# dyouakim/smpl

Hardware: AMD Instinct MI355X
Metric: successor evaluations/sec, ManipLattice GetSuccs loop body (7-DOF arm, 256^3 voxel grid) (higher is better)
Workload: dtype f64; 1 GPU; cfg2: 7-DOF arm7, 256^3 grid @ 0.02 m, tabletop + 64 boxes (seed 2), frontier batch B=4096 open states x M=25 primitives, eps 5 ARA* frontier; fork semantics (xy rotation by state[3]); batch_states=4096, primitives=25, grid=256, queries=1, parallelism=single query

## Files before the change

### smpl_amd/capi.py

```python
from __future__ import annotations

import ctypes as C
import os

import numpy as np

from . import build as _build

_dp = C.POINTER(C.c_double)
_ip = C.POINTER(C.c_int32)
_up = C.POINTER(C.c_uint8)
_u64p = C.POINTER(C.c_uint64)

SYMBOLS = [
    "smplx_last_error", "smplx_device_count", "smplx_shard_range", "smplx_grid_create", "smplx_grid_destroy", "smplx_model_create",
    "smplx_model_destroy", "smplx_model_counts", "smplx_model_joints", "smplx_model_nodes", "smplx_model_pairs",
    "smplx_space_create", "smplx_space_destroy", "smplx_space_num_vars", "smplx_space_num_prims",
    "smplx_space_discretization", "smplx_cc_state_valid_batch", "smplx_cc_edge_valid_batch", "smplx_cc_interpolate",
    "smplx_cc_sphere_positions", "smplx_set_goal_joint", "smplx_set_goal_xyz", "smplx_goal_pose",
    "smplx_heuristic_batch", "smplx_bfs_size", "smplx_bfs_copy", "smplx_bfs_levels", "smplx_expand_batch",
    "smplx_expand_work_bytes", "smplx_expand_batch_device", "smplx_set_start", "smplx_start_id", "smplx_goal_id",
    "smplx_get_succs", "smplx_hint_frontier", "smplx_get_goal_heuristic", "smplx_num_states", "smplx_get_state",
    "smplx_plan", "smplx_expansion_log_size", "smplx_expansion_log", "smplx_extract_path", "smplx_post_process_path", "smplx_space_specialized", "smplx_model_const_header", "smplx_profile_begin",
    "smplx_profile_end", "smplx_counters_bytes", "smplx_counters_read", "smplx_plan_multi",
# ... 566 lines not shown
        lib().smplx_test_set_one_launch.argtypes = [C.c_void_p, C.c_int]
        _chk(lib().smplx_test_set_one_launch(self.h, int(mode)))

    def one_launch_steps(self):
        lib().smplx_test_one_launch_steps.argtypes = [C.c_void_p]
        lib().smplx_test_one_launch_steps.restype = C.c_longlong
        return int(lib().smplx_test_one_launch_steps(self.h))

    def step_counters_zero(self, stream=None):
        lib().smplx_test_step_counters_zero.argtypes = [C.c_void_p, C.c_void_p]
        r = lib().smplx_test_step_counters_zero(self.h, C.c_void_p(stream))
        if r < 0:
            _chk(r)
        return r == 1

    def set_search_capacity(self, states):
        lib().smplx_test_set_search_capacity.argtypes = [C.c_void_p, C.c_int]
        _chk(lib().smplx_test_set_search_capacity(self.h, int(states)))

    def plan(self, eps0, eps_final, eps_delta, improve=True, bounded=False, max_init=0, max_rep=0, cap=100000):
        P = SearchParams(eps0, eps_final, eps_delta, int(improve), int(bounded), max_init, max_rep)
        S = SearchStats()
        ids = np.zeros(cap, np.int32)
        _chk(lib().smplx_plan(self.h, C.byref(P), _p(ids, _ip), cap, C.byref(S)))
        n = lib().smplx_expansion_log_size(self.h)
        log = np.zeros(n, np.int32)
        if n:
            _chk(lib().smplx_expansion_log(self.h, _p(log, _ip)))
        out = {f: getattr(S, f) for f, _ in SearchStats._fields_}
        out["path"] = ids[:S.path_len].copy()
# ... 83 lines not shown
```

### smpl_amd/csrc/device_table.h

```cpp
#pragma once

#include <cstring>
#include <vector>

#include "kernels.h"
#include "space.h"

namespace {

int table_alloc(smplx_space* s, size_t cap)
{
    if (s->dt.d_table) (void)hipFree(s->dt.d_table);
    s->dt.d_table = nullptr;
    const int stride = smplx_table_stride(s->N);
    HIP_TRY(hipMalloc((void**)&s->dt.d_table, cap * (size_t)stride * sizeof(int32_t)));
    HIP_TRY(hipMemsetAsync(s->dt.d_table, 0, cap * (size_t)stride * sizeof(int32_t), s->stream));
    s->dt.cap = cap;
    s->hs.table.slots = s->dt.d_table;
    s->hs.table.mask = (uint32_t)(cap - 1);
    s->hs.table.stride = stride;
    s->hs.table.pad = 0;
    return SMPLX_OK;
}

// ... 36 lines not shown
{
    if (items.empty()) return SMPLX_OK;
    const int n = (int)(items.size() / ((size_t)lead->N + 2));
    if (int e = dbuf.reserve(items.size())) return e;
    if (int e = pbuf.reserve(items.size())) return e;
    std::memcpy(pbuf.p, items.data(), items.size() * sizeof(int32_t));
    HIP_TRY(hipMemcpyAsync(dbuf.p, pbuf.p, items.size() * sizeof(int32_t), hipMemcpyHostToDevice, stream));
    hipLaunchKernelGGL(k_table_insert, dim3(blocks_for(n, SMPLX_BLOCK)), dim3(SMPLX_BLOCK), 0, stream, lead->d_space, stab, dbuf.p, n, lead->N);
    HIP_TRY(hipGetLastError());
    return SMPLX_OK;
}

int table_ensure(smplx_space* s)
{
    if (s->dt.d_table) return SMPLX_OK;
    size_t cap = (size_t)1 << 18;
    const size_t nstates = s->lat.h_of_id.size();
    while (nstates * 2 > cap) cap *= 4;
    if (int e = table_realloc(s, cap)) return e;
    s->dt.count = nstates > 0 ? nstates - 1 : 0;
    return SMPLX_OK;
}

int table_flush(smplx_space* s, hipStream_t stream)
{
    if (!s->dt.d_table) return SMPLX_OK;
    if (int e = table_grow_if_needed(s)) return e;
    if (s->dt.pending_ins.empty()) return SMPLX_OK;
    std::vector<int32_t> items;
    table_take_pending(s, 0, items);
    return table_upload(s, items, s->dt.b_ins, s->dt.p_ins, stream, nullptr);
// ... 4 lines not shown
```

### smpl_amd/csrc/engine.hip

```cpp
#include <hip/hip_runtime.h>

#include <algorithm>
#include <chrono>
#include <cmath>
#include <cstdlib>
#include <cstring>
#include <functional>
#include <limits>
#include <memory>
#include <string>
#include <vector>

#include "../../include/smpl_amd.h"
#include "det_math.h"
#include "device_types.h"
#include "kernels.h"
#include "model_compile.h"
#include "specialize.h"
#include "test_hooks.h"
#include "host_core.h"
#include "grid_handle.h"
#include "lattice.h"
#include "space.h"
#include "bfs_host.h"
// ... 350 lines not shown
long long smplx_test_one_launch_steps(const smplx_space* s) { return s ? (long long)s->step.one_launch_steps : -1; }

int smplx_test_step_counters_zero(smplx_space* s, void* stream)
{
    if (!s) return set_error(SMPLX_E_ARG, "null space");
    for (StepLaunch::WorkCounters& w : s->step.work_counters) {
        if (w.stream != (hipStream_t)stream) continue;
        std::vector<int32_t> h(SMPLX_WORK_COUNTER_BYTES / sizeof(int32_t));
        HIP_TRY(hipStreamSynchronize(w.stream));
        HIP_TRY(hipMemcpy(h.data(), w.p, SMPLX_WORK_COUNTER_BYTES, hipMemcpyDeviceToHost));
        for (int32_t v : h) if (v != 0) return 0;
        return 1;
    }
    return set_error(SMPLX_E_ARG, "no step has run on this stream");
}

int smplx_test_set_search_helper(smplx_space* s, int on)
{
    if (!s) return set_error(SMPLX_E_ARG, "null space");
    s->ds.test_no_helper = on == 0;
    return SMPLX_OK;
}

int smplx_test_set_search_capacity(smplx_space* s, int states)
{
    if (!s || states < 0) return set_error(SMPLX_E_ARG, "bad argument");
    s->ds.test_capacity = states;
    return SMPLX_OK;
}

// ... 1116 lines not shown
```

### smpl_amd/csrc/kernels.h

```cpp
#pragma once

#ifndef __HIPCC_RTC__
#include <hip/hip_runtime.h>
#include <stdint.h>
#endif

#include "device_types.h"

#define SMPLX_BLOCK 128
#define SMPLX_SETUP_BLOCK (SMPLX_BLOCK + 64)
#define SMPLX_STEP_BLOCK SMPLX_SETUP_BLOCK
#define SMPLX_STEP_STATES 16
#define SMPLX_STEP_CTR_BASE 512
#define SMPLX_STEP_CTR_OVERFLOW (SMPLX_STEP_CTR_BASE + 64 * SMPLX_CMP_SHARDS)
#define SMPLX_STEP_CTR_DONE (SMPLX_STEP_CTR_OVERFLOW + 32)
#define SMPLX_WORK_COUNTER_BYTES 16384
#define SMPLX_SEARCH_STATIC_LDS (44 * 1024)
#define SMPLX_GLOBAL_AS __attribute__((address_space(1)))
#define SMPLX_TALLIES 6

static inline int smplx_small_block(int nprims) { return ((nprims * 7 + 1) + 63) / 64 * 64 + 64; }
static inline int smplx_search_block(int nprims) { const int b = smplx_small_block(nprims); return b + 64 <= 512 ? b + 64 : b; }
static inline size_t smplx_lds_bytes_n(size_t blob_bytes, int nroot, int nslots, int nvars, int stack_bytes, int nthreads)
{
    return blob_bytes + (size_t)(3 * nroot + 12 * nslots + nvars) * 8 * nthreads + (size_t)stack_bytes * nthreads;
}
static inline size_t smplx_lds_bytes(size_t blob_bytes, int nroot, int nslots, int nvars, int stack_bytes)
{
    return smplx_lds_bytes_n(blob_bytes, nroot, nslots, nvars, stack_bytes, SMPLX_BLOCK);
}

static inline int smplx_step_states(int nprims) { return (SMPLX_BLOCK - 2 + nprims) / nprims + 1; }

#define SMPLX_PER_ROBOT_KERNELS(X) \
    X(STATE_PREP, k_state_prep) X(EXPAND, k_expand) X(PIPE_PREP, k_pipe_prep) X(PIPE_SETUP, k_pipe_setup) \
    X(PIPE_CONFIGS, k_pipe_configs) X(PIPE_FINISH, k_pipe_finish) X(SMALL_BATCH, k_small_batch) X(EDGE_VALID, k_edge_valid) \
    X(STATE_VALID, k_state_valid) X(HEURISTIC, k_heuristic) X(SPHERE_POSITIONS, k_sphere_positions) X(SEARCH, k_search) \
    X(ATTACHED_POSITIONS, k_attached_positions) X(PLANNING_POSE, k_planning_pose) X(STEP_BLOCK, k_step_block)

extern "C" {
__global__ void k_state_prep(const SmplxSpaceDev* S, const double* Q, int B, double* goal_dist,
                             unsigned char* parent_valid, int* parent_lookups,
                         const SmplxSpaceDev* const* stab, const unsigned short* state_q);
__global__ void k_expand(const SmplxSpaceDev* S, const double* Q, int B, const double* goal_dist,
                         const unsigned char* parent_valid, const int* parent_lookups, unsigned char* out_flags,
                         int* out_coord, double* out_q, int* out_h, int* out_cost, int* out_lookups,
                         unsigned long long* counters, const int* deferred_count,
// ... 59 lines not shown
```

### smpl_amd/csrc/lattice_steps.h

```cpp
#pragma once

#include "bfs_record.h"
#include "model_lds.h"
#include "sphere_checks.h"

__device__ __forceinline__ void planning_fk(const ModelLds* __restrict__ M, const double* __restrict__ q, double p[3], double* R)
{
    double T[12];
#pragma unroll
    for (int i = 0; i < 12; ++i) T[i] = 0.0;
#ifdef SMPLX_CONST_MODEL
    const_planning_chain<0, true>(M, q, T);
#else
    bool first = true;
    const int nj = M->njoints;
    for (int j = 0; j < nj; ++j) {
        JointPtr jt = &M->joints[j];
        if (!jt->on_chain) continue;
        double qv = 0.0;
        if (jt->var >= 0) {
            qv = q[jt->var];
            if (MV_TYPE(M, jt->var) == SMPLX_JT_CONTINUOUS) qv = smplx_normalize_angle(qv);
        }
        apply_joint(jt, qv, T, first);
// ... 108 lines not shown
}

__device__ __forceinline__ int var_to_coord(const ModelLds* __restrict__ M, int v, double x)
{
    const double delta = MV_COORD_DELTA(M, v);
    const int ty = MV_TYPE(M, v);
    if (ty == SMPLX_JT_CONTINUOUS) {
        const double pos = smplx_normalize_angle_positive(x);
        int c = (int)((pos + delta * 0.5) / delta);
        if (c == MV_COORD_VALS(M, v)) c = 0;
        return c;
    }
    return (int)(((x - MV_MIN(M, v)) / delta) + 0.5);
}

template <bool ConcurrentInserts>
__device__ __forceinline__ int table_lookup(const SmplxTableDev& T, const int* __restrict__ c, int nv)
{
    if (!T.slots) return -1;
    unsigned int i = smplx_coord_hash(c, nv) & T.mask;
    while (true) {
        const SMPLX_GLOBAL_AS int* sl = as_global(T.slots) + (size_t)i * T.stride;
        const int tag = ConcurrentInserts ? __atomic_load_n(&sl[0], __ATOMIC_ACQUIRE) : __atomic_load_n(&sl[0], __ATOMIC_RELAXED);
        if (tag <= 0) return -1;
        bool same = true;
        for (int v = 0; v < nv; ++v) same = same && (ConcurrentInserts ? __atomic_load_n(&sl[1 + v], __ATOMIC_RELAXED) : sl[1 + v]) == c[v];
        if (same) return tag - 1;
        i = (i + 1) & T.mask;
    }
}

__device__ __forceinline__ void table_insert_item(const SmplxSpaceDev* __restrict__ S, const SmplxSpaceDev* const* __restrict__ stab,
                                                  const int* __restrict__ it, int nvars)
{
    const SmplxTableDev T = (stab ? stab[it[0]] : S)->table;
    if (!T.slots) return;
    const int id = it[1];
    int c[SMPLX_MAX_VARS];
    for (int v = 0; v < nvars; ++v) c[v] = it[2 + v];
    unsigned int k = smplx_coord_hash(c, nvars) & T.mask;
    while (true) {
// ... 19 lines not shown
{
    if ((int)blockIdx.x < first_block) return false;
    const int i = ((int)blockIdx.x - first_block) * (int)blockDim.x + (int)threadIdx.x;
    const int nvars = S->model.nvars;
    if (i < n) table_insert_item(S, stab, items + (size_t)i * (nvars + 2), nvars);
    return true;
}

extern "C" __global__ void __launch_bounds__(BLOCK)
k_table_insert(const SmplxSpaceDev* __restrict__ S, const SmplxSpaceDev* const* __restrict__ stab, const int* __restrict__ items,
               int n, int nvars)
{
    table_insert_items(S, stab, items, n, nvars);
}

__device__ __forceinline__ bool mprim_active(const SmplxActionsDev& A, double goal_dist, int type)
{
    if (type == SMPLX_MP_LONG) {
        if (A.use_long_and_short) return true;
        const bool near_goal = goal_dist <= A.thresh[SMPLX_MP_SHORT];
        return !(A.enabled[SMPLX_MP_SHORT] && near_goal);
    } else if (type == SMPLX_MP_SHORT) {
        if (A.use_long_and_short) return A.enabled[type] != 0;
        const bool near_goal = goal_dist <= A.thresh[type];
        return A.enabled[type] && near_goal;
    }
    return A.enabled[type] && goal_dist <= A.thresh[type];
}

__device__ __forceinline__ bool prim_has_action(const SmplxActionsDev& A, const SmplxGoalDev& G, int p)
{
    const int ty = A.type[p];
    return ty == SMPLX_MP_LONG || ty == SMPLX_MP_SHORT || (ty == SMPLX_MP_SNAP_XYZ_RPY && G.type == SMPLX_GOAL_JOINT);
}

__device__ __forceinline__ bool successor_values(const ModelLds* __restrict__ M, const SmplxActionsDev& A, const SmplxGoalDev& G,
                                                 int pi, const double* __restrict__ parent, double* __restrict__ sq)
{
    const int nv = MV_NVARS(M);
    const int type = A.type[pi];
    if (type == SMPLX_MP_LONG || type == SMPLX_MP_SHORT) {
        double d0 = A.delta[pi][0], d1 = nv > 1 ? A.delta[pi][1] : 0.0;
// ... 54 lines not shown
```

### smpl_amd/csrc/search_kernel.h

```cpp
#pragma once

#include "small_batch.h"

#define SMPLX_AC_LEVELS 16
#define SMPLX_AC_SLOTS 128
#define SMPLX_INFINITECOST 1000000000u

enum { SA_EVAL = 0, SA_SKIP = 1, SA_REORDER = 2, SA_EXIT = 3 };

struct SearchLds {
    int action;
    int buf;
    int seq;
    int helper_gave_up;
    int go;
    double reorder_eps;
    int reorder_size, reorder_dups;
    int ac_nlev;
    int ac_lo[SMPLX_AC_LEVELS + 1], ac_hi[SMPLX_AC_LEVELS + 1], ac_base[SMPLX_AC_LEVELS + 1];
    unsigned long long ac_val[SMPLX_AC_SLOTS];
};

typedef unsigned long long hent_t;
#define HENT_ABSENT (~0ull)
// ... 182 lines not shown
    return h;
}

__device__ __forceinline__ void sstate_reinit(SmplxSState& s, int call_number)
{
    s.g = SMPLX_INFINITECOST;
    s.f = SMPLX_INFINITECOST;
    s.eg = SMPLX_INFINITECOST;
    s.iteration_closed = 0;
    s.call_number = (unsigned short)call_number;
    s.bp = -1;
    s.heap_index = 0;
    s.flags = 0;
}

typedef int __attribute__((ext_vector_type(4))) sk_int4;

__device__ __forceinline__ void sstate_store(SMPLX_GLOBAL_AS SmplxSState* dst, const SmplxSState& s, bool with_heap_index)
{
    sk_int4 a;
    a.x = (int)s.g; a.y = (int)s.h; a.z = (int)s.f; a.w = (int)s.eg;
    *(SMPLX_GLOBAL_AS sk_int4*)dst = a;
    dst->bp = s.bp;
    if (with_heap_index) dst->heap_index = s.heap_index;
    *(SMPLX_GLOBAL_AS unsigned int*)&dst->iteration_closed = (unsigned int)s.iteration_closed | ((unsigned int)s.call_number << 16);
    dst->flags = s.flags;
}
__device__ __forceinline__ SmplxSState sstate_load(const SMPLX_GLOBAL_AS SmplxSState* src)
{
    const sk_int4 a = ((const SMPLX_GLOBAL_AS sk_int4*)src)[0], b = ((const SMPLX_GLOBAL_AS sk_int4*)src)[1];
    SmplxSState s;
    s.g = (unsigned int)a.x; s.h = (unsigned int)a.y; s.f = (unsigned int)a.z; s.eg = (unsigned int)a.w;
    s.bp = b.x; s.heap_index = b.y;
    s.iteration_closed = (unsigned short)((unsigned int)b.z & 0xFFFFu); s.call_number = (unsigned short)((unsigned int)b.z >> 16);
    s.flags = (unsigned int)b.w;
    return s;
}

struct TableProbe { int id; unsigned int free_slot; };
#define SMPLX_TABLE_WORDS ((SMPLX_MAX_VARS + 1 + 3) / 4)
static_assert(4 * SMPLX_TABLE_WORDS >= SMPLX_MAX_VARS + 1, "the words of a probe hold the tag and every coordinate of the widest robot");
static_assert(4 * SMPLX_TABLE_WORDS <= (SMPLX_MAX_VARS + 1 + 7) / 8 * 8, "... and lie inside its slot (smplx_table_stride)");
struct TableProbeLoads { sk_int4 w[SMPLX_TABLE_WORDS]; unsigned int slot; };
__device__ __forceinline__ void table_slot_load(const SmplxTableDev& T, unsigned int slot, int nv, sk_int4 w[SMPLX_TABLE_WORDS])
{
    const SMPLX_GLOBAL_AS sk_int4* sl = (const SMPLX_GLOBAL_AS sk_int4*)(as_global(T.slots) + (size_t)slot * T.stride);
    const int nw = (nv + 1 + 3) / 4;
#pragma unroll
    for (int k = 0; k < SMPLX_TABLE_WORDS; ++k) if (k < nw) w[k] = sl[k];
}
__device__ __forceinline__ bool table_slot_match(const sk_int4 w[SMPLX_TABLE_WORDS], const LDS_AS int* c, int nv)
{
    const int nw = (nv + 1 + 3) / 4;
    bool same = w[0].x > 0;
#pragma unroll
    for (int k = 0; k < SMPLX_TABLE_WORDS; ++k) {
        if (k >= nw) continue;
        const int base = 4 * k - 1;
        if (k > 0 && base < nv) same = same && w[k].x == c[base];
        if (base + 1 < nv) same = same && w[k].y == c[base + 1];
        if (base + 2 < nv) same = same && w[k].z == c[base + 2];
        if (base + 3 < nv) same = same && w[k].w == c[base + 3];
    }
    return same;
}
__device__ __forceinline__ TableProbeLoads table_probe_start(const SmplxTableDev& T, int nv, unsigned int hash)
{
    TableProbeLoads r;
    r.slot = hash & T.mask;
    table_slot_load(T, r.slot, nv, r.w);
    return r;
}
__device__ __forceinline__ TableProbe table_probe_finish(const SmplxTableDev& T, TableProbeLoads& ld, const LDS_AS int* c, int nv)
{
    TableProbe r;
    while (true) {
        if (ld.w[0].x == 0) { r.id = -1; r.free_slot = ld.slot; return r; }
        if (table_slot_match(ld.w, c, nv)) { r.id = ld.w[0].x - 1; r.free_slot = 0; return r; }
        ld.slot = (ld.slot + 1) & T.mask;
        table_slot_load(T, ld.slot, nv, ld.w);
    }
}
__device__ __forceinline__ void table_store_own(const SmplxTableDev& T, unsigned int slot, const LDS_AS int* c, int nv, int id)
{
    SMPLX_GLOBAL_AS int* sl = as_global(T.slots) + (size_t)slot * T.stride;
    for (int v = 0; v < nv; ++v) sl[1 + v] = c[v];
    sl[0] = id + 1;
}

__device__ __forceinline__ bool ancestor_cache_fill(const HeapRef& H, SearchLds& W, int lane, int n, int cnt)
{
    int nlev = 0, total = 0;
    int my_idx[2] = {-1, -1};
// ... 871 lines not shown
```

### smpl_amd/csrc/space.h

```cpp
#pragma once

#include <chrono>
#include <cstdint>
#include <memory>
#include <string>
#include <utility>
#include <vector>

#include "device_types.h"
#include "grid_handle.h"
#include "host_core.h"
#include "lattice.h"
#include "model_compile.h"
#include "specialize.h"

namespace {

struct OutView {
    double* sq = nullptr;
    int32_t* coord = nullptr;
    int32_t* h = nullptr;
    int32_t* id = nullptr;
    unsigned char* flags = nullptr;
    size_t bytes = 0;
// ... 18 lines not shown
    DevBuf<unsigned char> b_work, b_out;
    DevBuf<int32_t> b_cost, b_lookups;
    PinBuf<double> p_q;
    PinBuf<unsigned short> p_stateq;
    PinBuf<unsigned char> p_out;
    std::vector<int32_t> ins_items;
    OutView dv, pv;
    hipEvent_t done = nullptr;
    bool zero_copy = false;
    std::chrono::steady_clock::time_point t_issue;
};

struct DeviceTable {
    int32_t* d_table = nullptr;
    size_t cap = 0, count = 0;
    int64_t regrows = 0;
    std::vector<int32_t> pending_ins;
    DevBuf<int32_t> b_ins;
    PinBuf<int32_t> p_ins;
};

struct BfsHost {
    int32_t* d_dist = nullptr;
    int32_t* d_queue = nullptr;
    int32_t* d_counts = nullptr;
    int32_t* d_brick_queued = nullptr;
    int bricks[3] = {0, 0, 0};
    int64_t total = 0;
    int64_t ints = 0;
    bool reset_due = false;
// ... 166 lines not shown
```

### smpl_amd/csrc/step.h

```cpp
#pragma once

#include <algorithm>
#include <chrono>
#include <cstddef>
#include <cstdlib>
#include <cstring>
#include <functional>
#include <string>
#include <utility>
#include <vector>

#include "device_table.h"
#include "kernels.h"
#include "space.h"

namespace {

inline size_t counter_words(int B, int M) { return (size_t)blocks_for((long long)B * M, SMPLX_BLOCK) * SMPLX_TALLIES; }

struct ExpandWork {
    double* goal_dist;
    int32_t* state_lookups;
    unsigned char* state_bad;
    int32_t* edge_w;
// ... 81 lines not shown
inline size_t small_lds_bytes(const smplx_space* s)
{
    return smplx_lds_bytes_n(s->blob_bytes, s->lds_nroot, s->model.dev.nslots, s->model.dev.nvars, s->model.dev.stack_bytes,
                             smplx_small_block(s->M));
}

ExpandPath expand_path(const smplx_space* s, int B, int zero_copy_max, bool force_pipeline)
{
    const bool small = !s->step.fused_mode && B <= s->small.batch_max && smplx_small_block(s->M) <= 512 &&
                       small_lds_bytes(s) <= 150 * 1024 && s->step.work_list_items == 0 && s->small.pipeline_left == 0 &&
                       s->step.prof_used + 3 > s->step.prof_events.size();
    if (small && B <= zero_copy_max && s->step.prof_events.empty()) return ExpandPath::SmallZeroCopy;
    if (small && !force_pipeline) return ExpandPath::Small;
    if (s->step.fused_mode) return ExpandPath::Fused;
    const bool can_run = s->step.one_launch_blocks > 0 && !s->step.pipe_prep && s->step.work_list_items == 0 &&
                         s->step.prof_used + 3 > s->step.prof_events.size();
    const bool by_rule = s->ks.specialized && s->step.one_launch_per_cu >= 4 &&
                         blocks_for((long long)B * s->M, SMPLX_BLOCK) <= s->step.one_launch_blocks;
    if (can_run && s->step.one_launch != 0 && (s->step.one_launch == 1 || by_rule)) return ExpandPath::OneLaunch;
    return ExpandPath::Pipeline;
}

int step_block_resident(const smplx_space* s, size_t lds, int* blocks_per_cu)
{
    *blocks_per_cu = 0;
    if (smplx_step_states(s->M) > SMPLX_STEP_STATES) return 0;
    int per_cu = 0, cus = 0;
    const smplx::KernelRef& k = s->ks.k[smplx::K_STEP_BLOCK];
    const hipError_t e = k.fn ? hipModuleOccupancyMaxActiveBlocksPerMultiprocessor(&per_cu, k.fn, SMPLX_STEP_BLOCK, lds)
                              : hipOccupancyMaxActiveBlocksPerMultiprocessor(&per_cu, k.generic, SMPLX_STEP_BLOCK, lds);
    if (e != hipSuccess) { (void)hipGetLastError(); return 0; }
// ... 15 lines not shown
    *out = &s->step.work_counters.back();
    return SMPLX_OK;
}

int launch_expand(smplx_space* s, const ExpandArgs& a)
{
    const int B = a.B;
    ExpandWork k = carve_work(a.work, B, s->M, s->N);
    int32_t* d_id = a.k5 ? a.k5->d_id : nullptr;
    SmplxCompactDev cmp;
    std::memset(&cmp, 0, sizeof(cmp));
    if (a.k5 && a.k5->cmp) cmp = *a.k5->cmp;
    const ExpandPath path = expand_path(s, B, a.zero_copy ? B : 0, a.force_pipeline || cmp.rec_a);
    if (s->step.one_launch == 1 && path == ExpandPath::Pipeline)
        return set_error(SMPLX_E_ARG, "the one-launch step was asked for (smplx_test_set_one_launch) but cannot run: a pipeline test hook or a "
                                      "profile-event triple is set, or a block of k_step_block does not fit this model");
    const int32_t* ins_items = a.k5 && s->dt.d_table ? a.k5->items : nullptr;
    const int n_ins = ins_items ? a.k5->n_items : 0;
    if (s->step.work_list_items > 0) k.capacity = s->step.work_list_items;
    hipEvent_t* ev = nullptr;
    if (s->step.prof_used + 3 <= s->step.prof_events.size()) { ev = &s->step.prof_events[s->step.prof_used]; s->step.prof_used += 3; }
    const int bs = blocks_for(B, SMPLX_BLOCK);
    const int be = blocks_for((long long)B * s->M, SMPLX_BLOCK);
    if (path == ExpandPath::SmallZeroCopy || path == ExpandPath::Small) {
        ++s->small.small_launches;
        const ZeroCopy* zc = path == ExpandPath::SmallZeroCopy ? a.zero_copy : nullptr;
        const int small_block = smplx_small_block(s->M);
        KLAUNCH(s, K_SMALL_BATCH, k_small_batch, dim3(B + blocks_for(n_ins, small_block)), dim3(small_block), small_lds_bytes(s), a.stream, s->d_space,
                           zc ? zc->q : a.q, B, k.goal_dist,
                           k.state_bad, k.state_lookups, a.flags, a.coord, a.sq, a.h, a.cost, a.lookups, a.stab, a.state_q,
                           zc ? zc->flags : (unsigned char*)nullptr, zc ? zc->coord : (int32_t*)nullptr,
// ... 361 lines not shown
```

### smpl_amd/csrc/step_block.h

```cpp
#pragma once

#include "step_kernels.h"

extern "C" __global__ void __launch_bounds__(SMPLX_STEP_BLOCK)
k_step_block(const SmplxSpaceDev* __restrict__ S, const double* __restrict__ Q, int B,
             unsigned char* __restrict__ out_flags, int* out_coord, double* out_q,
             int* __restrict__ out_h, int* __restrict__ out_cost, int* __restrict__ out_lookups,
             unsigned long long* __restrict__ counters,
        const SmplxSpaceDev* const* __restrict__ stab, const unsigned short* __restrict__ state_q,
             int* __restrict__ out_id, SmplxCompactDev cmp, int* __restrict__ step_ctr, int nprims, int nvars,
             const unsigned char* __restrict__ blob, int blob_bytes)
{
    extern __shared__ __align__(16) unsigned char smem[];
    constexpr int NT = SMPLX_STEP_BLOCK;
#ifdef SMPLX_CONST_MODEL
    constexpr bool RS = true;
#else
    constexpr bool RS = false;
#endif
    __shared__ double s_gd[SMPLX_STEP_STATES];
    __shared__ int s_slk[SMPLX_STEP_STATES], s_sbad[SMPLX_STEP_STATES];
    __shared__ int s_W[BLOCK], s_pre[BLOCK], s_elk[BLOCK], s_ebad[BLOCK];
    __shared__ int s_wsum[BLOCK / 64];
#ifdef SMPLX_CONST_MODEL
// ... 6 lines not shown
    const SmplxActionsDev& A = S->actions;
    const int nv = ARG_NVARS(nvars);
    const long long n_edges = (long long)B * nprims;
    const long long e0 = (long long)blockIdx.x * BLOCK;
    const long long e1 = e0 + BLOCK - 1 < n_edges ? e0 + BLOCK - 1 : n_edges - 1;
    const int s0 = (int)(e0 / nprims), s1 = (int)(e1 / nprims);
    const int n_states = s1 - s0 + 1;
    const bool dist_wave = t >= BLOCK;
    const int l = t - BLOCK;
    const long long tid = e0 + t;
    const bool in_range = !dist_wave && tid < n_edges;
    const int si = in_range ? (int)(tid / nprims) : s0;
    const int pi = in_range ? (int)(tid - (long long)si * nprims) : 0;
    const int ks = si - s0;
    const SmplxSpaceDev* Sq = stab ? stab[state_q[si]] : S;
    const int type = A.type[pi];
    if (t < BLOCK) { s_elk[t] = 0; s_ebad[t] = 0; }
    if (t < SMPLX_STEP_STATES) { s_slk[t] = 0; s_sbad[t] = 0; }
#ifdef SMPLX_CONST_MODEL
    double pqv[CM_NV], sqv[CM_NV];
#pragma unroll
    for (int v = 0; v < CM_NV; ++v) { pqv[v] = 0.0; sqv[v] = 0.0; }
    if (in_range) {
#pragma unroll
        for (int v = 0; v < CM_NV; ++v) pqv[v] = Q[(int64_t)si * CM_NV + v];
    }
    for (int i = t; i < n_states * CM_NV; i += NT) s_pq[i] = Q[(int64_t)s0 * CM_NV + i];
#endif
    ModelLds Mv;
    ThreadLds L = setup_lds(S, smem, &Mv, NT, !RS, blob, blob_bytes, fetched);
    const ModelLds* M = &Mv;
    const SmplxGridDev grid = S->grid;
    int W = 0;
    int flags = SMPLX_F_INACTIVE;
    int succ_h = 0, succ_id = -1;
    bool succ_goal = false;
#ifdef SMPLX_CONST_MODEL
    int scv[CM_NV];
#pragma unroll
    for (int v = 0; v < CM_NV; ++v) scv[v] = 0;
    if (in_range) flags = pipe_edge_values(M, A, Sq, pi, pqv, sqv, W);
    if (dist_wave) {
        if constexpr (CM_PARENT_TRIG) {
            constexpr int PER = 64 / CM_NV;
            const int ls = l / CM_NV, lv = l - ls * CM_NV;
            for (int r0 = 0; r0 < n_states; r0 += PER) {
                const int k = r0 + ls;
                double ns = 0.0, nc = 0.0;
                if (ls < PER && k < n_states) {
                    const double x = s_pq[k * CM_NV + lv];
                    double rs = 0.0, rc = 0.0;
                    if ((CM_TRIG_ANY >> lv) & 1u) smplx_sincos(x, &rs, &rc);
                    ns = rs; nc = rc;
                    bool cont = false;
#pragma unroll
                    for (int u = 0; u < CM_NV; ++u) if (CM_VAR_TYPE[u] == SMPLX_JT_CONTINUOUS) cont = cont || lv == u;
// ... 25 lines not shown
            double qd[CM_NV];
#pragma unroll
            for (int v = 0; v < CM_NV; ++v) qd[v] = s_pq[l * CM_NV + v];
            s_gd[l] = metric_goal_distance(M, grid, bfs, qd);
        }
    }
#else
    if (dist_wave && l < n_states) {
        const SmplxBfsDev bfs = (stab ? stab[state_q[s0 + l]] : S)->bfs;
        s_gd[l] = metric_goal_distance(M, grid, bfs, Q + (int64_t)(s0 + l) * nv);
    }
#endif
    __syncthreads();
    int items = 0;
    if (in_range) {
        if (!mprim_active(A, s_gd[ks], type)) {
            flags = SMPLX_F_INACTIVE;
            W = 0;
        } else {
#ifdef SMPLX_CONST_MODEL
            if (flags != SMPLX_F_INACTIVE) {
#pragma unroll
                for (int v = 0; v < CM_NV; ++v) { s_sq[v * BLOCK + t] = sqv[v]; out_q[tid * CM_NV + v] = sqv[v]; }
            }
#ifndef ABL_NO_SUCC
            if (flags == 0) {
                constexpr bool SC = CM_PARENT_TRIG && CM_TRIG_PLANNING != 0;
                if constexpr (SC) {
                    double prow[2 * CM_NV], sn[CM_NV], cs[CM_NV];
#pragma unroll
                    for (int j = 0; j < 2 * CM_NV; ++j) prow[j] = s_trig[ks * SMPLX_TRIG_ROW + 2 * CM_NV + j];
                    parent_trig<CM_TRIG_PLANNING, true>(sqv, pqv, prow, sn, cs);
                    pipe_successor<true>(M, Sq, grid, sqv, scv, out_id != nullptr, succ_h, succ_id, succ_goal, sn, cs);
                } else {
                    pipe_successor(M, Sq, grid, sqv, scv, out_id != nullptr, succ_h, succ_id, succ_goal);
                }
            }
#endif
#else
            flags = pipe_edge_values(M, A, Sq, pi, Q + (int64_t)si * nv, out_q + tid * nv, W);
#endif
        }
        items = W > 0 ? W - 1 : 0;
    }
    const int lane = t & 63, wv = t >> 6;
    int incl = items;
    for (int off = 1; off < 64; off <<= 1) {
        const int u = __shfl_up(incl, off);
        if (lane >= off) incl += u;
    }
    if (!dist_wave) {
// ... 95 lines not shown
#endif
                h = succ_h;
                cost = A.cost[pi];
                flags = SMPLX_F_VALID | (succ_goal ? SMPLX_F_GOAL : 0);
            }
        } else {
            succ_id = -1;
        }
        out_flags[tid] = (unsigned char)flags;
        out_h[tid] = h;
        out_cost[tid] = cost;
        out_lookups[tid] = lookups;
        succ_h = h;
        if (out_id) out_id[tid] = succ_id;
    }
    if (cmp.rec_a) {
        __shared__ int c_cnt[BLOCK / 64][2];
        __shared__ int c_base[2];
        const bool is_a = in_range && (flags & SMPLX_F_VALID) != 0;
        const bool is_b = is_a && (succ_id < 0 || (flags & SMPLX_F_GOAL) != 0);
        const unsigned long long m_a = __ballot(is_a), m_b = __ballot(is_b);
        const unsigned long long below = lane == 0 ? 0ull : (~0ull >> (64 - lane));
        if (lane == 0 && !dist_wave) { c_cnt[wv][0] = __popcll(m_a); c_cnt[wv][1] = __popcll(m_b); }
        __syncthreads();
        if (t == 0) {
            int ta = 0, tb = 0;
#pragma unroll
            for (int k = 0; k < BLOCK / 64; ++k) { ta += c_cnt[k][0]; tb += c_cnt[k][1]; }
            const int shard = blockIdx.x % SMPLX_CMP_SHARDS;
            const int sa = cmp.cap_a / SMPLX_CMP_SHARDS, sb = cmp.cap_b / SMPLX_CMP_SHARDS;
            int ba = ta > 0 ? atomicAdd(&step_ctr[SMPLX_STEP_CTR_BASE + 64 * shard], ta) : 0;
            int bb = tb > 0 ? atomicAdd(&step_ctr[SMPLX_STEP_CTR_BASE + 64 * shard + 32], tb) : 0;
            if (ba + ta > sa || bb + tb > sb) {
                atomicExch(&step_ctr[SMPLX_STEP_CTR_OVERFLOW], 1);
                __threadfence();
                ba = -1;
            }
            else { ba += shard * sa; bb += shard * sb; }
            c_base[0] = ba; c_base[1] = bb;
            int* bt = cmp.block_tab + 4 * (size_t)blockIdx.x;
            bt[0] = ba; bt[1] = ta; bt[2] = bb; bt[3] = tb;
        }
        __syncthreads();
        if (c_base[0] >= 0 && is_a) {
            int ia = c_base[0] + __popcll(m_a & below), ib = c_base[1] + __popcll(m_b & below);
            for (int k = 0; k < wv; ++k) { ia += c_cnt[k][0]; ib += c_cnt[k][1]; }
            cmp.rec_a[2 * (size_t)ia] = succ_id;
            cmp.rec_a[2 * (size_t)ia + 1] = pi | ((flags & SMPLX_F_GOAL) ? 0x100 : 0) | (si << 9);
            if (is_b) {
                unsigned char* rb = cmp.rec_b + (size_t)ib * cmp.rec_b_bytes;
                int* ri = (int*)rb;
                double* rq = (double*)(rb + (size_t)((nv + 2) / 2 * 2) * 4);
                ri[0] = succ_h;
#ifdef SMPLX_CONST_MODEL
#pragma unroll
                for (int v = 0; v < CM_NV; ++v) { ri[1 + v] = scv[v]; rq[v] = s_sq[v * BLOCK + t]; }
#else
                for (int v = 0; v < nv; ++v) { ri[1 + v] = out_coord[tid * nv + v]; rq[v] = out_q[tid * nv + v]; }
#endif
            }
        }
    }
    if (counters) {
        const unsigned long long m_eval = __ballot(evaluated);
        const unsigned long long m_valid = __ballot((flags & SMPLX_F_VALID) != 0);
        tally_block<NT / 64>(counters, dist_wave ? 0 : __popcll(m_eval), dist_wave ? 0 : __popcll(m_valid), lookups, performed, ncfg, slk);
    }
    if (cmp.rec_a) {
        __shared__ int s_last;
        if (t == 0) {
            const int nb = (int)gridDim.x, shard = blockIdx.x % SMPLX_CMP_SHARDS;
            const int in_shard = (nb - shard + SMPLX_CMP_SHARDS - 1) / SMPLX_CMP_SHARDS;
            const int shards = nb < SMPLX_CMP_SHARDS ? nb : SMPLX_CMP_SHARDS;
            int last = 0;
            if (atomicAdd(&step_ctr[SMPLX_STEP_CTR_DONE + 32 * (1 + shard)], 1) == in_shard - 1)
                last = atomicAdd(&step_ctr[SMPLX_STEP_CTR_DONE], 1) == shards - 1 ? 1 : 0;
            s_last = last;
        }
        __syncthreads();
        if (s_last) {
            if (t < 2 * SMPLX_CMP_SHARDS) {
                const int shard = t >> 1, region = t & 1;
                cmp.totals[32 * shard + region] = atomicExch(&step_ctr[SMPLX_STEP_CTR_BASE + 64 * shard + 32 * region], 0);
            } else if (t == 2 * SMPLX_CMP_SHARDS) {
                cmp.totals[32 * SMPLX_CMP_SHARDS] = atomicExch(&step_ctr[SMPLX_STEP_CTR_OVERFLOW], 0);
            } else if (t <= 2 * SMPLX_CMP_SHARDS + 1 + SMPLX_CMP_SHARDS) {
                atomicExch(&step_ctr[SMPLX_STEP_CTR_DONE + 32 * (t - 2 * SMPLX_CMP_SHARDS - 1)], 0);
            }
        }
    }
}
```

### smpl_amd/csrc/step_kernels.h

```cpp
#pragma once

#include "config_checks.h"
#include "lattice_steps.h"


extern "C" __global__ void __launch_bounds__(BLOCK, 2)
k_state_prep(const SmplxSpaceDev* __restrict__ S, const double* __restrict__ Q, int B,
             double* __restrict__ goal_dist, unsigned char* __restrict__ parent_valid, int* __restrict__ parent_lookups,
        const SmplxSpaceDev* const* __restrict__ stab, const unsigned short* __restrict__ state_q)
{
    extern __shared__ __align__(16) unsigned char smem[];
    ModelLds Mv;
    ThreadLds L = setup_lds(S, smem, &Mv);
    const ModelLds* M = &Mv;
    const SmplxGridDev grid = S->grid;
    const int i = blockIdx.x * BLOCK + threadIdx.x;
    if (i >= B) return;
    const SmplxBfsDev bfs = (stab ? stab[state_q[i]] : S)->bfs;
    const double* q = Q + (int64_t)i * MV_NVARS(M);
    goal_dist[i] = metric_goal_distance(M, grid, bfs, q);
    EdgeRef e;
    e.start = q; e.finish = q; e.alpha = 0.0;
    int lk = 0;
    const bool ok = config_valid(M, L, grid, e, lk);
// ... 317 lines not shown
            unsigned long long* wl = work + (size_t)shard * shard_cap;
            if (first + items <= shard_cap && W <= SMPLX_WP_MAX) {
                const unsigned long long base = (unsigned long long)tid | ((unsigned long long)W << 48);
                for (int k = 0; k < items; ++k) wl[first + k] = base | ((unsigned long long)(k + 1) << 32);
            } else {
                for (int k = first; k < first + items && k < shard_cap; ++k) wl[k] = SMPLX_WORK_BLANK;
                flags = SMPLX_F_DEFERRED;
                atomicAdd(&work_count[SMPLX_WORK_SHARDS * SMPLX_SHARD_STRIDE], 1);
            }
        }
        edge_w[tid] = W;
        out_flags[tid] = (unsigned char)flags;
    }
}

template <bool SC = false>
__device__ __forceinline__ void pipe_successor(const ModelLds* __restrict__ M, const SmplxSpaceDev* __restrict__ Sq,
                                               const SmplxGridDev& grid, const double* __restrict__ sq, int* __restrict__ sc,
                                               bool want_id, int& h, int& id, bool& is_goal, const double* sn = nullptr,
                                               const double* cs = nullptr)
{
    const int nv = MV_NVARS(M);
    const SmplxBfsDev bfs = Sq->bfs;
    MV_UNROLL
    for (int v = 0; v < nv; ++v) sc[v] = var_to_coord(M, v, sq[v]);
    id = want_id ? table_lookup<false>(Sq->table, sc, nv) : -1;
    h = successor_goal_h<SC>(M, Sq->goal, bfs, grid, sq, sc, is_goal, sn, cs);
}

__device__ __forceinline__ void pipe_successor_role(const SmplxSpaceDev* __restrict__ S, int B, int cfg_blocks,
                                                    const unsigned char* __restrict__ out_flags, const double* __restrict__ out_q,
                                                    int* __restrict__ succ_coord, const SmplxSpaceDev* const* __restrict__ stab,
                                                    const unsigned short* __restrict__ state_q, bool want_id,
                                                    unsigned long long* __restrict__ succ_eval, unsigned char* __restrict__ succ_goal,
                                                    unsigned char* smem, int nprims, int nvars,
                                                    const double* __restrict__ Q, const double* __restrict__ trig)
{
    const long long tid = (long long)((int)blockIdx.x - cfg_blocks) * BLOCK + threadIdx.x;
    const bool live = tid < (long long)B * nprims && out_flags[tid] == 0;
#ifdef SMPLX_CONST_MODEL
    double qv[CM_NV];
    if (live) {
// ... 312 lines not shown
```

Before: 1.923 billion successor evaluations/s.

## Issue table probe before heuristic, pack compaction claim counters into one atomic

The successor hash-table probe now loads the home slot as vector words before the goal heuristic is computed and resolves it afterwards, so the table load latency can overlap the heuristic work. The per-shard compaction claim counters for the two regions and the block-done count are packed into one 64-bit atomic, which removes separate atomics and the fence in the block epilogue. The motion-primitive gate is hoisted, and successor coordinates are computed earlier. Packing adds a limit on counter width, guarded by a fit check that falls back to the pipeline path, and it adds test hooks for the table size.

```diff
diff --git a/smpl_amd/capi.py b/smpl_amd/capi.py
--- a/smpl_amd/capi.py
+++ b/smpl_amd/capi.py
@@ -604,6 +604,15 @@
             _chk(r)
         return r == 1
 
+    def set_table_slots(self, slots):
+        lib().smplx_test_set_table_slots.argtypes = [C.c_void_p, C.c_int]
+        _chk(lib().smplx_test_set_table_slots(self.h, int(slots)))
+
+    def table_slots(self):
+        lib().smplx_test_table_slots.argtypes = [C.c_void_p]
+        lib().smplx_test_table_slots.restype = C.c_longlong
+        return int(lib().smplx_test_table_slots(self.h))
+
     def set_search_capacity(self, states):
         lib().smplx_test_set_search_capacity.argtypes = [C.c_void_p, C.c_int]
         _chk(lib().smplx_test_set_search_capacity(self.h, int(states)))
diff --git a/smpl_amd/csrc/device_table.h b/smpl_amd/csrc/device_table.h
--- a/smpl_amd/csrc/device_table.h
+++ b/smpl_amd/csrc/device_table.h
@@ -74,7 +74,7 @@
 int table_ensure(smplx_space* s)
 {
     if (s->dt.d_table) return SMPLX_OK;
-    size_t cap = (size_t)1 << 18;
+    size_t cap = s->dt.test_slots ? s->dt.test_slots : (size_t)1 << 18;
     const size_t nstates = s->lat.h_of_id.size();
     while (nstates * 2 > cap) cap *= 4;
     if (int e = table_realloc(s, cap)) return e;
diff --git a/smpl_amd/csrc/engine.hip b/smpl_amd/csrc/engine.hip
--- a/smpl_amd/csrc/engine.hip
+++ b/smpl_amd/csrc/engine.hip
@@ -388,6 +388,16 @@
     }
     return set_error(SMPLX_E_ARG, "no step has run on this stream");
 }
+
+int smplx_test_set_table_slots(smplx_space* s, int slots)
+{
+    if (!s || slots < 0 || (slots != 0 && (slots < 64 || (slots & (slots - 1)) != 0)))
+        return set_error(SMPLX_E_ARG, "slots must be 0 or a power of two of at least 64");
+    s->dt.test_slots = (size_t)slots;
+    return SMPLX_OK;
+}
+
+long long smplx_test_table_slots(const smplx_space* s) { return s ? (long long)(s->dt.d_table ? s->dt.cap : 0) : -1; }
 
 int smplx_test_set_search_helper(smplx_space* s, int on)
 {
diff --git a/smpl_amd/csrc/kernels.h b/smpl_amd/csrc/kernels.h
--- a/smpl_amd/csrc/kernels.h
+++ b/smpl_amd/csrc/kernels.h
@@ -12,8 +12,9 @@
 #define SMPLX_STEP_BLOCK SMPLX_SETUP_BLOCK
 #define SMPLX_STEP_STATES 16
 #define SMPLX_STEP_CTR_BASE 512
-#define SMPLX_STEP_CTR_OVERFLOW (SMPLX_STEP_CTR_BASE + 64 * SMPLX_CMP_SHARDS)
-#define SMPLX_STEP_CTR_DONE (SMPLX_STEP_CTR_OVERFLOW + 32)
+#define SMPLX_STEP_CTR_DONE (SMPLX_STEP_CTR_BASE + 32 * SMPLX_CMP_SHARDS)
+#define SMPLX_STEP_CLAIM_BITS 24
+#define SMPLX_STEP_COUNT_BITS 16
 #define SMPLX_WORK_COUNTER_BYTES 16384
 #define SMPLX_SEARCH_STATIC_LDS (44 * 1024)
 #define SMPLX_GLOBAL_AS __attribute__((address_space(1)))
@@ -31,6 +32,11 @@
 }
 
 static inline int smplx_step_states(int nprims) { return (SMPLX_BLOCK - 2 + nprims) / nprims + 1; }
+static inline bool smplx_step_claim_fits(long long blocks)
+{
+    const long long in_shard = (blocks + SMPLX_CMP_SHARDS - 1) / SMPLX_CMP_SHARDS;
+    return in_shard < (1ll << SMPLX_STEP_COUNT_BITS) && in_shard * SMPLX_BLOCK < (1ll << SMPLX_STEP_CLAIM_BITS);
+}
 
 #define SMPLX_PER_ROBOT_KERNELS(X) \
     X(STATE_PREP, k_state_prep) X(EXPAND, k_expand) X(PIPE_PREP, k_pipe_prep) X(PIPE_SETUP, k_pipe_setup) \
diff --git a/smpl_amd/csrc/lattice_steps.h b/smpl_amd/csrc/lattice_steps.h
--- a/smpl_amd/csrc/lattice_steps.h
+++ b/smpl_amd/csrc/lattice_steps.h
@@ -146,17 +146,75 @@
     return (int)(((x - MV_MIN(M, v)) / delta) + 0.5);
 }
 
+#define SMPLX_TABLE_WORDS ((SMPLX_MAX_VARS + 1 + 3) / 4)
+static_assert(4 * SMPLX_TABLE_WORDS >= SMPLX_MAX_VARS + 1, "the words of a probe hold the tag and every coordinate of the widest robot");
+static_assert(4 * SMPLX_TABLE_WORDS <= (SMPLX_MAX_VARS + 1 + 7) / 8 * 8, "... and lie inside its slot (smplx_table_stride)");
+typedef int __attribute__((ext_vector_type(4))) table_int4;
+struct TableSlotWords { table_int4 w[SMPLX_TABLE_WORDS]; unsigned int slot; };
+
+__device__ __forceinline__ void table_slot_load(const SmplxTableDev& T, unsigned int slot, int nv, table_int4 w[SMPLX_TABLE_WORDS])
+{
+    const SMPLX_GLOBAL_AS table_int4* sl = (const SMPLX_GLOBAL_AS table_int4*)(as_global(T.slots) + (size_t)slot * T.stride);
+    const int nw = (nv + 1 + 3) / 4;
+#pragma unroll
+    for (int k = 0; k < SMPLX_TABLE_WORDS; ++k) if (k < nw) w[k] = sl[k];
+}
+template <class CoordPtr>
+__device__ __forceinline__ bool table_slot_match(const table_int4 w[SMPLX_TABLE_WORDS], CoordPtr c, int nv)
+{
+    const int nw = (nv + 1 + 3) / 4;
+    int differ = 0;
+#pragma unroll
+    for (int k = 0; k < SMPLX_TABLE_WORDS; ++k) {
+        if (k >= nw) continue;
+        const int base = 4 * k - 1;
+        if (k > 0 && base < nv) differ |= w[k].x ^ c[base];
+        if (base + 1 < nv) differ |= w[k].y ^ c[base + 1];
+        if (base + 2 < nv) differ |= w[k].z ^ c[base + 2];
+        if (base + 3 < nv) differ |= w[k].w ^ c[base + 3];
+    }
+    return differ == 0;
+}
+
+__device__ __forceinline__ TableSlotWords table_probe_none()
+{
+    TableSlotWords r;
+#pragma unroll
+    for (int k = 0; k < SMPLX_TABLE_WORDS; ++k) r.w[k] = table_int4{0, 0, 0, 0};
+    r.slot = 0;
+    return r;
+}
+__device__ __forceinline__ TableSlotWords table_probe_issue(const SmplxTableDev& T, const int* __restrict__ c, int nv)
+{
+    TableSlotWords r = table_probe_none();
+    if (!T.slots) return r;
+    r.slot = smplx_coord_hash(c, nv) & T.mask;
+    table_slot_load(T, r.slot, nv, r.w);
+    return r;
+}
+__device__ __forceinline__ int table_probe_resolve(const SmplxTableDev& T, const int* __restrict__ c, int nv, TableSlotWords ld)
+{
+    while (true) {
+        const int tag = ld.w[0].x;
+        if (tag <= 0) return -1;
+        if (table_slot_match(ld.w, c, nv)) return tag - 1;
+        ld.slot = (ld.slot + 1) & T.mask;
+        table_slot_load(T, ld.slot, nv, ld.w);
+    }
+}
+
 template <bool ConcurrentInserts>
 __device__ __forceinline__ int table_lookup(const SmplxTableDev& T, const int* __restrict__ c, int nv)
 {
+    if constexpr (!ConcurrentInserts) return table_probe_resolve(T, c, nv, table_probe_issue(T, c, nv));
     if (!T.slots) return -1;
     unsigned int i = smplx_coord_hash(c, nv) & T.mask;
     while (true) {
         const SMPLX_GLOBAL_AS int* sl = as_global(T.slots) + (size_t)i * T.stride;
-        const int tag = ConcurrentInserts ? __atomic_load_n(&sl[0], __ATOMIC_ACQUIRE) : __atomic_load_n(&sl[0], __ATOMIC_RELAXED);
+        const int tag = __atomic_load_n(&sl[0], __ATOMIC_ACQUIRE);
         if (tag <= 0) return -1;
         bool same = true;
-        for (int v = 0; v < nv; ++v) same = same && (ConcurrentInserts ? __atomic_load_n(&sl[1 + v], __ATOMIC_RELAXED) : sl[1 + v]) == c[v];
+        for (int v = 0; v < nv; ++v) same = same && __atomic_load_n(&sl[1 + v], __ATOMIC_RELAXED) == c[v];
         if (same) return tag - 1;
         i = (i + 1) & T.mask;
     }
@@ -206,18 +264,27 @@
     table_insert_items(S, stab, items, n, nvars);
 }
 
+struct MprimGate { int type, use_long_and_short, enabled; double thresh; };
+__device__ __forceinline__ MprimGate mprim_gate(const SmplxActionsDev& A, int type)
+{
+    const int kind = type == SMPLX_MP_LONG ? SMPLX_MP_SHORT : type;
+    MprimGate g;
+    g.type = type;
+    g.use_long_and_short = A.use_long_and_short;
+    g.enabled = A.enabled[kind];
+    g.thresh = A.thresh[kind];
+    return g;
+}
+__device__ __forceinline__ bool mprim_active(const MprimGate& g, double goal_dist)
+{
+    const bool near_goal = goal_dist <= g.thresh;
+    if (g.type == SMPLX_MP_LONG) return g.use_long_and_short || !(g.enabled && near_goal);
+    if (g.type == SMPLX_MP_SHORT && g.use_long_and_short) return g.enabled != 0;
+    return g.enabled && near_goal;
+}
 __device__ __forceinline__ bool mprim_active(const SmplxActionsDev& A, double goal_dist, int type)
 {
-    if (type == SMPLX_MP_LONG) {
-        if (A.use_long_and_short) return true;
-        const bool near_goal = goal_dist <= A.thresh[SMPLX_MP_SHORT];
-        return !(A.enabled[SMPLX_MP_SHORT] && near_goal);
-    } else if (type == SMPLX_MP_SHORT) {
-        if (A.use_long_and_short) return A.enabled[type] != 0;
-        const bool near_goal = goal_dist <= A.thresh[type];
-        return A.enabled[type] && near_goal;
-    }
-    return A.enabled[type] && goal_dist <= A.thresh[type];
+    return mprim_active(mprim_gate(A, type), goal_dist);
 }
 
 __device__ __forceinline__ bool prim_has_action(const SmplxActionsDev& A, const SmplxGoalDev& G, int p)
diff --git a/smpl_amd/csrc/search_kernel.h b/smpl_amd/csrc/search_kernel.h
--- a/smpl_amd/csrc/search_kernel.h
+++ b/smpl_amd/csrc/search_kernel.h
@@ -220,7 +220,7 @@
     s.flags = 0;
 }
 
-typedef int __attribute__((ext_vector_type(4))) sk_int4;
+typedef table_int4 sk_int4;
 
 __device__ __forceinline__ void sstate_store(SMPLX_GLOBAL_AS SmplxSState* dst, const SmplxSState& s, bool with_heap_index)
 {
@@ -244,32 +244,7 @@
 }
 
 struct TableProbe { int id; unsigned int free_slot; };
-#define SMPLX_TABLE_WORDS ((SMPLX_MAX_VARS + 1 + 3) / 4)
-static_assert(4 * SMPLX_TABLE_WORDS >= SMPLX_MAX_VARS + 1, "the words of a probe hold the tag and every coordinate of the widest robot");
-static_assert(4 * SMPLX_TABLE_WORDS <= (SMPLX_MAX_VARS + 1 + 7) / 8 * 8, "... and lie inside its slot (smplx_table_stride)");
-struct TableProbeLoads { sk_int4 w[SMPLX_TABLE_WORDS]; unsigned int slot; };
-__device__ __forceinline__ void table_slot_load(const SmplxTableDev& T, unsigned int slot, int nv, sk_int4 w[SMPLX_TABLE_WORDS])
-{
-    const SMPLX_GLOBAL_AS sk_int4* sl = (const SMPLX_GLOBAL_AS sk_int4*)(as_global(T.slots) + (size_t)slot * T.stride);
-    const int nw = (nv + 1 + 3) / 4;
-#pragma unroll
-    for (int k = 0; k < SMPLX_TABLE_WORDS; ++k) if (k < nw) w[k] = sl[k];
-}
-__device__ __forceinline__ bool table_slot_match(const sk_int4 w[SMPLX_TABLE_WORDS], const LDS_AS int* c, int nv)
-{
-    const int nw = (nv + 1 + 3) / 4;
-    bool same = w[0].x > 0;
-#pragma unroll
-    for (int k = 0; k < SMPLX_TABLE_WORDS; ++k) {
-        if (k >= nw) continue;
-        const int base = 4 * k - 1;
-        if (k > 0 && base < nv) same = same && w[k].x == c[base];
-        if (base + 1 < nv) same = same && w[k].y == c[base + 1];
-        if (base + 2 < nv) same = same && w[k].z == c[base + 2];
-        if (base + 3 < nv) same = same && w[k].w == c[base + 3];
-    }
-    return same;
-}
+typedef TableSlotWords TableProbeLoads;
 __device__ __forceinline__ TableProbeLoads table_probe_start(const SmplxTableDev& T, int nv, unsigned int hash)
 {
     TableProbeLoads r;
@@ -282,7 +257,7 @@
     TableProbe r;
     while (true) {
         if (ld.w[0].x == 0) { r.id = -1; r.free_slot = ld.slot; return r; }
-        if (table_slot_match(ld.w, c, nv)) { r.id = ld.w[0].x - 1; r.free_slot = 0; return r; }
+        if (ld.w[0].x > 0 && table_slot_match(ld.w, c, nv)) { r.id = ld.w[0].x - 1; r.free_slot = 0; return r; }
         ld.slot = (ld.slot + 1) & T.mask;
         table_slot_load(T, ld.slot, nv, ld.w);
     }
diff --git a/smpl_amd/csrc/space.h b/smpl_amd/csrc/space.h
--- a/smpl_amd/csrc/space.h
+++ b/smpl_amd/csrc/space.h
@@ -56,6 +56,7 @@
 struct DeviceTable {
     int32_t* d_table = nullptr;
     size_t cap = 0, count = 0;
+    size_t test_slots = 0;
     int64_t regrows = 0;
     std::vector<int32_t> pending_ins;
     DevBuf<int32_t> b_ins;
diff --git a/smpl_amd/csrc/step.h b/smpl_amd/csrc/step.h
--- a/smpl_amd/csrc/step.h
+++ b/smpl_amd/csrc/step.h
@@ -119,7 +119,8 @@
     if (small && !force_pipeline) return ExpandPath::Small;
     if (s->step.fused_mode) return ExpandPath::Fused;
     const bool can_run = s->step.one_launch_blocks > 0 && !s->step.pipe_prep && s->step.work_list_items == 0 &&
-                         s->step.prof_used + 3 > s->step.prof_events.size();
+                         s->step.prof_used + 3 > s->step.prof_events.size() &&
+                         smplx_step_claim_fits(blocks_for((long long)B * s->M, SMPLX_BLOCK));
     const bool by_rule = s->ks.specialized && s->step.one_launch_per_cu >= 4 &&
                          blocks_for((long long)B * s->M, SMPLX_BLOCK) <= s->step.one_launch_blocks;
     if (can_run && s->step.one_launch != 0 && (s->step.one_launch == 1 || by_rule)) return ExpandPath::OneLaunch;
@@ -165,7 +166,8 @@
     const ExpandPath path = expand_path(s, B, a.zero_copy ? B : 0, a.force_pipeline || cmp.rec_a);
     if (s->step.one_launch == 1 && path == ExpandPath::Pipeline)
         return set_error(SMPLX_E_ARG, "the one-launch step was asked for (smplx_test_set_one_launch) but cannot run: a pipeline test hook or a "
-                                      "profile-event triple is set, or a block of k_step_block does not fit this model");
+                                      "profile-event triple is set, a block of k_step_block does not fit this model, or the grid is beyond "
+                                      "what its claim words count");
     const int32_t* ins_items = a.k5 && s->dt.d_table ? a.k5->items : nullptr;
     const int n_ins = ins_items ? a.k5->n_items : 0;
     if (s->step.work_list_items > 0) k.capacity = s->step.work_list_items;
diff --git a/smpl_amd/csrc/step_block.h b/smpl_amd/csrc/step_block.h
--- a/smpl_amd/csrc/step_block.h
+++ b/smpl_amd/csrc/step_block.h
@@ -44,7 +44,11 @@
     const int pi = in_range ? (int)(tid - (long long)si * nprims) : 0;
     const int ks = si - s0;
     const SmplxSpaceDev* Sq = stab ? stab[state_q[si]] : S;
-    const int type = A.type[pi];
+    const MprimGate gate = mprim_gate(A, A.type[pi]);
+#if defined(SMPLX_CONST_MODEL) && !defined(ABL_NO_SUCC)
+    SmplxTableDev table = {nullptr, 0u, 0, 0};
+    if (out_id) table = Sq->table;
+#endif
     if (t < BLOCK) { s_elk[t] = 0; s_ebad[t] = 0; }
     if (t < SMPLX_STEP_STATES) { s_slk[t] = 0; s_sbad[t] = 0; }
 #ifdef SMPLX_CONST_MODEL
@@ -70,6 +74,11 @@
 #pragma unroll
     for (int v = 0; v < CM_NV; ++v) scv[v] = 0;
     if (in_range) flags = pipe_edge_values(M, A, Sq, pi, pqv, sqv, W);
+#ifndef ABL_NO_SUCC
+    if (in_range && flags == 0) {
+        successor_coords(M, sqv, scv);
+    }
+#endif
     if (dist_wave) {
         if constexpr (CM_PARENT_TRIG) {
             constexpr int PER = 64 / CM_NV;
@@ -125,7 +134,7 @@
     __syncthreads();
     int items = 0;
     if (in_range) {
-        if (!mprim_active(A, s_gd[ks], type)) {
+        if (!mprim_active(gate, s_gd[ks])) {
             flags = SMPLX_F_INACTIVE;
             W = 0;
         } else {
@@ -137,15 +146,18 @@
 #ifndef ABL_NO_SUCC
             if (flags == 0) {
                 constexpr bool SC = CM_PARENT_TRIG && CM_TRIG_PLANNING != 0;
+                const SmplxBfsDev sbfs = Sq->bfs;
+                const TableSlotWords home = table_probe_issue(table, scv, CM_NV);
                 if constexpr (SC) {
                     double prow[2 * CM_NV], sn[CM_NV], cs[CM_NV];
 #pragma unroll
                     for (int j = 0; j < 2 * CM_NV; ++j) prow[j] = s_trig[ks * SMPLX_TRIG_ROW + 2 * CM_NV + j];
                     parent_trig<CM_TRIG_PLANNING, true>(sqv, pqv, prow, sn, cs);
-                    pipe_successor<true>(M, Sq, grid, sqv, scv, out_id != nullptr, succ_h, succ_id, succ_goal, sn, cs);
+                    succ_h = successor_goal_h<true>(M, Sq->goal, sbfs, grid, sqv, scv, succ_goal, sn, cs);
                 } else {
-                    pipe_successor(M, Sq, grid, sqv, scv, out_id != nullptr, succ_h, succ_id, succ_goal);
+                    succ_h = successor_goal_h(M, Sq->goal, sbfs, grid, sqv, scv, succ_goal);
                 }
+                succ_id = table_probe_resolve(table, scv, CM_NV, home);
             }
 #endif
 #else
@@ -271,6 +283,7 @@
         succ_h = h;
         if (out_id) out_id[tid] = succ_id;
     }
+    __shared__ int s_last;
     if (cmp.rec_a) {
         __shared__ int c_cnt[BLOCK / 64][2];
         __shared__ int c_base[2];
@@ -284,15 +297,20 @@
             int ta = 0, tb = 0;
 #pragma unroll
             for (int k = 0; k < BLOCK / 64; ++k) { ta += c_cnt[k][0]; tb += c_cnt[k][1]; }
-            const int shard = blockIdx.x % SMPLX_CMP_SHARDS;
+            const int nb = (int)gridDim.x, shard = blockIdx.x % SMPLX_CMP_SHARDS;
+            const int in_shard = (nb - shard + SMPLX_CMP_SHARDS - 1) / SMPLX_CMP_SHARDS;
+            const int shards = nb < SMPLX_CMP_SHARDS ? nb : SMPLX_CMP_SHARDS;
             const int sa = cmp.cap_a / SMPLX_CMP_SHARDS, sb = cmp.cap_b / SMPLX_CMP_SHARDS;
-            int ba = ta > 0 ? atomicAdd(&step_ctr[SMPLX_STEP_CTR_BASE + 64 * shard], ta) : 0;
-            int bb = tb > 0 ? atomicAdd(&step_ctr[SMPLX_STEP_CTR_BASE + 64 * shard + 32], tb) : 0;
-            if (ba + ta > sa || bb + tb > sb) {
-                atomicExch(&step_ctr[SMPLX_STEP_CTR_OVERFLOW], 1);
-                __threadfence();
-                ba = -1;
-            }
+            unsigned long long* word = reinterpret_cast<unsigned long long*>(step_ctr + SMPLX_STEP_CTR_BASE + 32 * shard);
+            const unsigned long long mine = (unsigned long long)ta | ((unsigned long long)tb << 24) | (1ull << 48);
+            const unsigned long long was = atomicAdd(word, mine);
+            const int ba0 = ta > 0 ? (int)(was & 0xFFFFFFull) : 0, bb0 = tb > 0 ? (int)((was >> 24) & 0xFFFFFFull) : 0;
+            int ba = ba0, bb = bb0;
+            int last = 0;
+            if ((int)(was >> 48) == in_shard - 1)
+                last = atomicAdd(&step_ctr[SMPLX_STEP_CTR_DONE], 1) == shards - 1 ? 1 : 0;
+            s_last = last;
+            if (ba + ta > sa || bb + tb > sb) ba = -1;
             else { ba += shard * sa; bb += shard * sb; }
             c_base[0] = ba; c_base[1] = bb;
             int* bt = cmp.block_tab + 4 * (size_t)blockIdx.x;
@@ -323,26 +341,17 @@
         const unsigned long long m_valid = __ballot((flags & SMPLX_F_VALID) != 0);
         tally_block<NT / 64>(counters, dist_wave ? 0 : __popcll(m_eval), dist_wave ? 0 : __popcll(m_valid), lookups, performed, ncfg, slk);
     }
-    if (cmp.rec_a) {
-        __shared__ int s_last;
-        if (t == 0) {
-            const int nb = (int)gridDim.x, shard = blockIdx.x % SMPLX_CMP_SHARDS;
-            const int in_shard = (nb - shard + SMPLX_CMP_SHARDS - 1) / SMPLX_CMP_SHARDS;
-            const int shards = nb < SMPLX_CMP_SHARDS ? nb : SMPLX_CMP_SHARDS;
-            int last = 0;
-            if (atomicAdd(&step_ctr[SMPLX_STEP_CTR_DONE + 32 * (1 + shard)], 1) == in_shard - 1)
-                last = atomicAdd(&step_ctr[SMPLX_STEP_CTR_DONE], 1) == shards - 1 ? 1 : 0;
-            s_last = last;
-        }
-        __syncthreads();
-        if (s_last) {
-            if (t < 2 * SMPLX_CMP_SHARDS) {
-                const int shard = t >> 1, region = t & 1;
-                cmp.totals[32 * shard + region] = atomicExch(&step_ctr[SMPLX_STEP_CTR_BASE + 64 * shard + 32 * region], 0);
-            } else if (t == 2 * SMPLX_CMP_SHARDS) {
-                cmp.totals[32 * SMPLX_CMP_SHARDS] = atomicExch(&step_ctr[SMPLX_STEP_CTR_OVERFLOW], 0);
-            } else if (t <= 2 * SMPLX_CMP_SHARDS + 1 + SMPLX_CMP_SHARDS) {
-                atomicExch(&step_ctr[SMPLX_STEP_CTR_DONE + 32 * (t - 2 * SMPLX_CMP_SHARDS - 1)], 0);
+    if (cmp.rec_a && s_last) {
+        if (t < SMPLX_CMP_SHARDS) {
+            unsigned long long* word = reinterpret_cast<unsigned long long*>(step_ctr + SMPLX_STEP_CTR_BASE + 32 * t);
+            const unsigned long long tot = atomicExch(word, 0ull);
+            const int na = (int)(tot & 0xFFFFFFull), nb = (int)((tot >> 24) & 0xFFFFFFull);
+            cmp.totals[32 * t] = na;
+            cmp.totals[32 * t + 1] = nb;
+            const unsigned long long over = __ballot(na > cmp.cap_a / SMPLX_CMP_SHARDS || nb > cmp.cap_b / SMPLX_CMP_SHARDS);
+            if (t == 0) {
+                cmp.totals[32 * SMPLX_CMP_SHARDS] = over != 0ull ? 1 : 0;
+                atomicExch(&step_ctr[SMPLX_STEP_CTR_DONE], 0);
             }
         }
     }
diff --git a/smpl_amd/csrc/step_kernels.h b/smpl_amd/csrc/step_kernels.h
--- a/smpl_amd/csrc/step_kernels.h
+++ b/smpl_amd/csrc/step_kernels.h
@@ -355,6 +355,13 @@
     }
 }
 
+__device__ __forceinline__ void successor_coords(const ModelLds* __restrict__ M, const double* __restrict__ sq, int* __restrict__ sc)
+{
+    const int nv = MV_NVARS(M);
+    MV_UNROLL
+    for (int v = 0; v < nv; ++v) sc[v] = var_to_coord(M, v, sq[v]);
+}
+
 template <bool SC = false>
 __device__ __forceinline__ void pipe_successor(const ModelLds* __restrict__ M, const SmplxSpaceDev* __restrict__ Sq,
                                                const SmplxGridDev& grid, const double* __restrict__ sq, int* __restrict__ sc,
@@ -363,10 +370,10 @@
 {
     const int nv = MV_NVARS(M);
     const SmplxBfsDev bfs = Sq->bfs;
-    MV_UNROLL
-    for (int v = 0; v < nv; ++v) sc[v] = var_to_coord(M, v, sq[v]);
-    id = want_id ? table_lookup<false>(Sq->table, sc, nv) : -1;
+    successor_coords(M, sq, sc);
+    const TableSlotWords home = want_id ? table_probe_issue(Sq->table, sc, nv) : table_probe_none();
     h = successor_goal_h<SC>(M, Sq->goal, bfs, grid, sq, sc, is_goal, sn, cs);
+    id = want_id ? table_probe_resolve(Sq->table, sc, nv, home) : -1;
 }
 
 __device__ __forceinline__ void pipe_successor_role(const SmplxSpaceDev* __restrict__ S, int B, int cfg_blocks,
```

After: 2.053 billion successor evaluations/s (median of 6 runs). +6.7%, better.
